# zju3dv/EnvGS

Hardware: AMD Instinct MI355X
Metric: train iters/s (fwd+bwd of the render hot path + Adam step, one 800x800 view per GPU per iter) + render Mpix/s (higher is better)
Workload: dtype f32

## Files before the change

### envgs_amd/csrc/trace_surfel_bwd.hip

```cpp
#include "trace_common.h"

namespace envgs {

#define ENVGS_LDS_FENCE() do { __builtin_amdgcn_s_waitcnt(0xc07f); __builtin_amdgcn_sched_barrier(0); } while (0)
#ifndef ENVGS_BS_GROUP
#define ENVGS_BS_GROUP 15
#endif
constexpr int BS_GROUP = ENVGS_BS_GROUP;
static_assert(BS_GROUP <= 16, "stage() assigns four lanes per entry");
#ifndef ENVGS_BSB_KO
#define ENVGS_BSB_KO 0
#endif

typedef float f32x4 __attribute__((ext_vector_type(4)));
constexpr int BT_PITCH = 96;
constexpr int RECW = 64;
template <bool RGBO, bool OTH>
__global__ void __attribute__((amdgpu_waves_per_eu(ENVGS_BSB_WAVES, ENVGS_BSB_WAVES))) __launch_bounds__(64)
batch_surfel_bwd(const TraceArgs A)
{
    static_assert(!(RGBO && OTH), "the colour-only form never touches `others`");
    __shared__ float4 sdat[2][BS_GROUP][16];
    __shared__ unsigned long long sdesc[2][BS_GROUP];
    __shared__ unsigned short kmat[2][BS_GROUP][64];
    __shared__ unsigned spb[2][BS_GROUP];
    __shared__ unsigned scn[2][BS_GROUP];
    __shared__ float btile[16][BT_PITCH];
    __shared__ float2 sox[2][BS_GROUP];
    const int lane = threadIdx.x;
    const int nb = (A.D + 1) * (A.D + 1);
    const int nbatch = (A.R + 63) >> 6;
    for (int slot = blockIdx.x; slot < nbatch; slot += gridDim.x) {
        const int batch = A.bwd_order ? (int)A.bwd_order[slot] : slot;
        if ((unsigned)batch >= (unsigned)nbatch) continue;
        const int base = batch << 6;
        const int copy = batch & (NCOPY - 1);
        const int r = ray_of(A, base + lane);
        const bool valid = r < A.R && A.hit_cnt[r < A.R ? r : 0] <= A.cap;
        const int rr = r < A.R ? r : 0;
        float basis[16], Box, Boy, Boz, Bdx, Bdy, Bdz, gR0, gR1, gR2, gD, gA, gN0, gN1, gN2, gX0, gX1, Fsum;
        {
            BwdRay B;
            bwd_load_ray(A, rr, B);
#pragma unroll
            for (int k = 0; k < 16; k++) basis[k] = 0.f;
            sh_basis(A.D, B.ux, B.uy, B.uz, basis);
            if (A.M == 0) basis[0] = kC0;
            if (!(B.il > 0.0f && B.il < 3.0e38f)) {
#pragma unroll
                for (int k = 0; k < 16; k++) basis[k] = 0.f;
            }
            Box = B.ox; Boy = B.oy; Boz = B.oz; Bdx = B.dx; Bdy = B.dy; Bdz = B.dz;
            gR0 = B.gR0; gR1 = B.gR1; gR2 = B.gR2;
            if constexpr (RGBO) { gD = gA = gN0 = gN1 = gN2 = gX0 = gX1 = 0.f; }
            else { gD = B.gD; gA = B.gA; gN0 = B.gN0; gN1 = B.gN1; gN2 = B.gN2; gX0 = B.gX0; gX1 = B.gX1; }
            Fsum = bwd_final_dot(B);
        }
        float Areg[16];
        __syncthreads();
#pragma unroll
        for (int k = 0; k < 16; k++) btile[k][lane + 2 * k] = (valid && k < nb) ? basis[k] : (k == 0 ? kC0 : 0.f);
        __syncthreads();
#pragma unroll
        for (int sI = 0; sI < 16; sI++) Areg[sI] = btile[lane & 15][4 * sI + (lane >> 4) + 2 * (lane & 15)];
        float Acol[16];
#pragma unroll
        for (int q = 0; q < 16; q++) {
            const int k = 4 * (q & 3) + (lane >> 4);
            Acol[q] = btile[k][16 * (q >> 2) + (lane & 15) + 2 * k];
        }
        __syncthreads();
        f32x4 SkM[4];
#pragma unroll
        for (int k = 0; k < 4; k++) SkM[k] = f32x4{0.f, 0.f, 0.f, 0.f};
        float dO0 = 0.f, dO1 = 0.f, dO2 = 0.f, dD0 = 0.f, dD1 = 0.f, dD2 = 0.f;
        const float4 *state = A.state + state_row0(A, min(base + lane, A.R - 1), rr);
        const char *plane1 = reinterpret_cast<const char *>(A.state + A.state_plane);
        size_t rstart, region;
        batch_region(A, batch, rstart, region);
        const unsigned long long *ent = A.entries + rstart;
        const unsigned *prs = A.pairs + rstart;
        const int D = A.n_entries[2 * batch], NE = D + A.n_entries[2 * batch + 1];
        unsigned poff = 0u;
        auto stage = [&](int g, int buf) {
            const int el = lane >> 2, part = lane & 3;
            const int e = g * BS_GROUP + el;
            const bool elv = el < BS_GROUP;
            unsigned long long d = 0ull;
            if (elv && e < NE) {
                d = e < D ? ent[e] : ent[region - 1 - (size_t)(e - D)];
                const int sid = (int)(d & 0xFFFFFFull);
                sdat[buf][el][part] = A.srec[(size_t)sid * 4 + part];
                if (A.M == 16 && A.f16) {
                    const uint2 *s2 = reinterpret_cast<const uint2 *>(reinterpret_cast<const __half *>(A.shs) + (size_t)sid * 48);
#pragma unroll
                    for (int q = 0; q < 3; q++) {
                        const uint2 h = s2[part * 3 + q];
                        float4 x = make_float4(__half2float(__ushort_as_half((unsigned short)(h.x & 0xFFFFu))), __half2float(__ushort_as_half((unsigned short)(h.x >> 16))),
                                               __half2float(__ushort_as_half((unsigned short)(h.y & 0xFFFFu))), __half2float(__ushort_as_half((unsigned short)(h.y >> 16))));
                        const int i0 = (part * 3 + q) * 4;
                        if (i0 + 0 >= nb * 3) x.x = 0.f;
                        if (i0 + 1 >= nb * 3) x.y = 0.f;
                        if (i0 + 2 >= nb * 3) x.z = 0.f;
                        if (i0 + 3 >= nb * 3) x.w = 0.f;
                        sdat[buf][el][4 + part * 3 + q] = x;
                    }
                } else if (A.M == 16) {
                    const float4 *s4 = reinterpret_cast<const float4 *>(A.shs + (size_t)sid * 48);
#pragma unroll
                    for (int q = 0; q < 3; q++) {
                        float4 x = s4[part * 3 + q];
                        const int i0 = (part * 3 + q) * 4;
                        if (i0 + 0 >= nb * 3) x.x = 0.f;
                        if (i0 + 1 >= nb * 3) x.y = 0.f;
                        if (i0 + 2 >= nb * 3) x.z = 0.f;
                        if (i0 + 3 >= nb * 3) x.w = 0.f;
                        sdat[buf][el][4 + part * 3 + q] = x;
                    }
                } else {
                    const Feat fsh = Feat{A.shs, A.f16 != 0}.at(A.M > 0 ? (size_t)sid * A.M * 3 : 0), fcol = Feat{A.colors, A.f16 != 0}.at(A.M > 0 ? 0 : (size_t)sid * 3);
#pragma unroll
                    for (int q = 0; q < 3; q++) {
                        float v[4];
#pragma unroll
                        for (int c = 0; c < 4; c++) {
                            const int idx = (part * 3 + q) * 4 + c;
                            v[c] = A.M > 0 ? (idx < nb * 3 ? fsh[idx] : 0.f) : (idx < 3 ? fcol[idx] : 0.f);
                        }
                        sdat[buf][el][4 + part * 3 + q] = make_float4(v[0], v[1], v[2], v[3]);
                    }
                }
                if (part == 0) {
                    const size_t ci = (size_t)sid * NCOPY + copy;
                    const unsigned rec = A.surf_off[ci] - A.surf_cnt[ci] + (unsigned)(d >> 32);
                    sdesc[buf][el] = (d & 0x3FFFFFFFull) | ((unsigned long long)rec << 32);
                    if constexpr (OTH) sox[buf][el] = reinterpret_cast<const float2 *>(A.others)[sid];
                }
            }
            if (part == 0 && elv) scn[buf][el] = e < NE ? (unsigned)((d >> 24) & 63ull) + 1u : 0u;
            if (lane * 32 < BS_GROUP * 128) {
                uint4 *km = reinterpret_cast<uint4 *>(&kmat[buf][0][0]);
                km[lane * 2] = make_uint4(0u, 0u, 0u, 0u); km[lane * 2 + 1] = make_uint4(0u, 0u, 0u, 0u);
            }
            __syncthreads();
            unsigned pref[BS_GROUP + 1];
            pref[0] = 0u;
#pragma unroll
            for (int q = 0; q < BS_GROUP; q++) pref[q + 1] = pref[q] + scn[buf][q];
            unsigned tab_before = 0u;
#pragma unroll
            for (int q = 0; q < BS_GROUP; q++) {
                const int eq = g * BS_GROUP + q;
                if (lane == q) spb[buf][q] = eq < D ? poff + tab_before : (unsigned)(region - 1 - (size_t)(eq - D));
                if (eq < D) tab_before += scn[buf][q];
            }
            __syncthreads();
            const unsigned total = pref[BS_GROUP];
            for (unsigned q = lane; q < total; q += 64) {
                int eli = 0;
#pragma unroll
                for (int t = 1; t < BS_GROUP; t++) eli += q >= pref[t] ? 1 : 0;
                const unsigned pr = prs[spb[buf][eli] + (q - pref[eli])];
                kmat[buf][eli][pr >> 16] = (unsigned short)((pr & 0xFFFFu) + 1u);
            }
            poff += tab_before;
        };
        __syncthreads();
        stage(0, 0);
        for (int g = 0; g * BS_GROUP < NE; g++) {
            const int buf = g & 1;
            __syncthreads();
            if ((g + 1) * BS_GROUP < NE) stage(g + 1, buf ^ 1);
            const int ne = min(BS_GROUP, NE - g * BS_GROUP);
            int k1 = valid ? (int)kmat[buf][0][lane] : 0;
            float4 st0, st1 = make_float4(0.f, 0.f, 0.f, 0.f), st2 = make_float4(0.f, 0.f, 0.f, 0.f);
            auto fetch_state = [&](const int k) {
                const float4 *sp = k > 0 ? state + (size_t)(k - 1) : A.state;
                if (ENVGS_BSB_KO & 8) st0 = make_float4(0.5f, 0.1f, 0.1f, 0.1f); else st0 = sp[0];
                if constexpr (!RGBO) {
                    if (ENVGS_BSB_KO & 4) return;
                    if constexpr (OTH) {
                        typedef float f3 __attribute__((ext_vector_type(3), aligned(4)));
                        const float *q = reinterpret_cast<const float *>(plane1 + (size_t)(sp - A.state) * 24);
                        const f3 a = *reinterpret_cast<const f3 *>(q); st1.x = a.x; st1.y = a.y; st1.z = a.z;
                        if (!(ENVGS_BSB_KO & 2)) { const f3 b = *reinterpret_cast<const f3 *>(q + 3); st1.w = b.x; st2.x = b.y; st2.y = b.z; }
                    } else st1 = *reinterpret_cast<const float4 *>(plane1 + (size_t)(sp - A.state) * 16);
                }
            };
            fetch_state(k1);
            auto entry = [&]<int e5>(const int el) __attribute__((always_inline)) {
                const unsigned long long d = sdesc[buf][el];
                const int sid = (int)(d & 0xFFFFFFull);
                const unsigned long long rec = d >> 32;
                const bool act = k1 > 0;
                float gw[16];
#pragma unroll
                for (int n = 0; n < 16; n++) gw[n] = 0.f;
                [[maybe_unused]] float gx1 = 0.f;
#define BT(n) btile[3 * e5 + (n)][lane + 2 * (3 * e5 + (n))]
                if (A.M > 0 && e5 == 0) {
                    const int nrun = min(5, ne - el);
                    const int kk = lane >> 4, nn = lane & 15, ee = nn / 3, c2 = nn - 3 * ee;
                    f32x4 cc0 = {0.f, 0.f, 0.f, 0.f}, cc1 = cc0, cc2 = cc0, cc3 = cc0;
                    float bvc[4];
#pragma unroll
                    for (int ks = 0; ks < 4; ks++) {
                        bvc[ks] = 0.f;
                        if (nn < 15 && ee < nrun) bvc[ks] = reinterpret_cast<const float *>(&sdat[buf][el + ee][4])[(4 * ks + kk) * 3 + c2];
                    }
                    ENVGS_LDS_FENCE();
#pragma unroll
                    for (int ks = 0; ks < 4; ks++) {
                        cc0 = __builtin_amdgcn_mfma_f32_16x16x4f32(Acol[ks], bvc[ks], cc0, 0, 0, 0);
                        cc1 = __builtin_amdgcn_mfma_f32_16x16x4f32(Acol[4 + ks], bvc[ks], cc1, 0, 0, 0);
                        cc2 = __builtin_amdgcn_mfma_f32_16x16x4f32(Acol[8 + ks], bvc[ks], cc2, 0, 0, 0);
                        cc3 = __builtin_amdgcn_mfma_f32_16x16x4f32(Acol[12 + ks], bvc[ks], cc3, 0, 0, 0);
                    }
                    if (nn < 15) {
                        float *trow = &btile[nn][0];
#pragma unroll
                        for (int i = 0; i < 4; i++) {
                            const int j = 4 * kk + i + 2 * nn;
                            trow[j] = cc0[i]; trow[j + 16] = cc1[i]; trow[j + 32] = cc2[i]; trow[j + 48] = cc3[i];
                        }
                    }
                }
                if (act) {
                    const float4 s0 = sdat[buf][el][0], s1 = sdat[buf][el][1], s2 = sdat[buf][el][2], s3 = sdat[buf][el][3];
                    const SurfHit h = hit_surfel(s0, s1, s2, s3, Box, Boy, Boz, Bdx, Bdy, Bdz);
                    float col[3]; bool cl[3] = {false, false, false};
                    if (A.M > 0) {
                        const float rc[3] = {BT(0), BT(1), BT(2)};
#pragma unroll
                        for (int c = 0; c < 3; c++) { const float v = rc[c] + 0.5f; cl[c] = v < 0.f; col[c] = cl[c] ? 0.f : v; }
                    } else { const float4 x = sdat[buf][el][4]; col[0] = x.x; col[1] = x.y; col[2] = x.z; }
                    float x0 = 0.f, x1 = 0.f;
                    if constexpr (OTH) { const float2 xo = sox[buf][el]; x0 = xo.x; x1 = xo.y; }
                    const float alpha = h.alpha, w = alpha * st0.x;
                    const float sgn = h.denom < 0.0f ? 1.0f : -1.0f;
                    const float nf0 = sgn * s3.x, nf1 = sgn * s3.y, nf2 = sgn * s3.z;
                    const float inv1m = __builtin_amdgcn_rcpf(1.0f - alpha);
                    const float dLa = alpha_grad_from_state(RGBO, gR0, gR1, gR2, gD, gA, gN0, gN1, gN2, gX0, gX1, Fsum, col, h.t, nf0, nf1, nf2, x0, x1,
                                                            alpha, inv1m, st0, st1, st2.x, st2.y);
                    if constexpr (OTH) { gw[15] = w * gX0; gx1 = w * gX1; }
                    BT(0) = cl[0] ? 0.f : w * gR0; BT(1) = cl[1] ? 0.f : w * gR1; BT(2) = cl[2] ? 0.f : w * gR2;
                    float e0, e1, e2;
                    hit_geometry_grad(s0, s1, s2, s3, h, Box, Boy, Boz, Bdx, Bdy, Bdz, w, sgn, dLa, gD, gN0, gN1, gN2, A.mod,
                                      __builtin_amdgcn_rcpf(s1.w), __builtin_amdgcn_rcpf(s2.w), __builtin_amdgcn_rcpf(h.denom), gw, e0, e1, e2);
                    dO0 += e0; dO1 += e1; dO2 += e2;
                    dD0 += h.t * e0; dD1 += h.t * e1; dD2 += h.t * e2;
                } else {
                    BT(0) = 0.f; BT(1) = 0.f; BT(2) = 0.f;
                }
#undef BT
                if (el + 1 < ne) {
                    k1 = valid ? (int)kmat[buf][el + 1][lane] : 0;
                    fetch_state(k1);
                }
                {
                    if constexpr (OTH && !(ENVGS_BSB_KO & 1)) {
                        float g20[20];
#pragma unroll
                        for (int n = 0; n < 20; n++) g20[n] = n < 15 ? gw[n] : 0.f;
                        g20[15] = gw[15]; g20[16] = gx1;
                        const float gsum = wave_transpose_reduce<5>(g20, lane);
                        const int word = (lane & 15) + 5 * (lane >> 4);
                        if ((lane & 15) < 5 && word < 15 && rec < A.num_records) A.records[rec * RECW + 48 + word] = gsum;
                        if ((lane & 15) < 5 && (word == 15 || word == 16) && A.dothers) atomic_add_f32(A.dothers + 2 * sid + (word - 15), gsum);
                    } else {
                        const float gsum = wave_transpose_reduce<4>(gw, lane);
                        const int word = (lane & 15) + 4 * (lane >> 4);
                        if ((lane & 15) < 4 && word < 15 && rec < A.num_records) A.records[rec * RECW + 48 + word] = gsum;
                    }
                }
                if (e5 == 4 || el + 1 == ne) {
                    f32x4 acc4 = {0.f, 0.f, 0.f, 0.f}, accB = acc4, accC = acc4, accD = acc4;
                    {
                        const int n = lane & 15, j = lane >> 4;
                        const float *brow = &btile[n][0];
                        const int rot = 2 * n + j;
                        float bvr[16];
#pragma unroll
                        for (int sI = 0; sI < 16; sI++) bvr[sI] = brow[4 * sI + rot];
                        ENVGS_LDS_FENCE();
#pragma unroll
                        for (int sI = 0; sI < 16; sI += 4) {
                            acc4 = __builtin_amdgcn_mfma_f32_16x16x4f32(Areg[sI], bvr[sI], acc4, 0, 0, 0);
                            accB = __builtin_amdgcn_mfma_f32_16x16x4f32(Areg[sI + 1], bvr[sI + 1], accB, 0, 0, 0);
                            accC = __builtin_amdgcn_mfma_f32_16x16x4f32(Areg[sI + 2], bvr[sI + 2], accC, 0, 0, 0);
                            accD = __builtin_amdgcn_mfma_f32_16x16x4f32(Areg[sI + 3], bvr[sI + 3], accD, 0, 0, 0);
                        }
                    }
                    acc4 = (acc4 + accB) + (accC + accD);
                    const int n = lane & 15, mrow = (lane >> 4) * 4, er = n / 3, cc = n - 3 * er;
                    if (n < 15 && er <= e5) {
                        const unsigned long long rc = sdesc[buf][el - e5 + er] >> 32;
                        if (rc < A.num_records) {
                            float *ro = A.records + rc * RECW;
                            if (A.M > 0) { ro[(mrow + 0) * 3 + cc] = acc4[0]; ro[(mrow + 1) * 3 + cc] = acc4[1]; ro[(mrow + 2) * 3 + cc] = acc4[2]; ro[(mrow + 3) * 3 + cc] = acc4[3]; }
                            else if (mrow == 0) ro[cc] = acc4[0] * (1.0f / kC0);
                        }
                    }
                    if (A.M > 0) {
                        const int kk = lane >> 4, nn = lane & 15;
                        float bvs[4], avs[16];
#pragma unroll
                        for (int ks = 0; ks < 4; ks++) {
                            const int col = 4 * ks + kk, ee = col / 3, c2 = col - 3 * ee;
                            bvs[ks] = 0.f;
                            if (col < 15 && ee <= e5) bvs[ks] = reinterpret_cast<const float *>(&sdat[buf][el - e5 + ee][4])[nn * 3 + c2];
                            const float *arow = &btile[col][0];
#pragma unroll
                            for (int rb = 0; rb < 4; rb++) avs[4 * ks + rb] = arow[16 * rb + nn + 2 * col];
                        }
                        ENVGS_LDS_FENCE();
#pragma unroll
                        for (int ks = 0; ks < 4; ks++)
#pragma unroll
                            for (int rb = 0; rb < 4; rb++)
                                SkM[rb] = __builtin_amdgcn_mfma_f32_16x16x4f32(avs[4 * ks + rb], bvs[ks], SkM[rb], 0, 0, 0);
                    }
                }
            };
            for (int el = 0; el < ne; el += 5) {
                entry.template operator()<0>(el);
                if (el + 1 >= ne) break;
                entry.template operator()<1>(el + 1);
                if (el + 2 >= ne) break;
                entry.template operator()<2>(el + 2);
                if (el + 3 >= ne) break;
                entry.template operator()<3>(el + 3);
                if (el + 4 >= ne) break;
                entry.template operator()<4>(el + 4);
            }
        }
        __syncthreads();
#pragma unroll
        for (int rb = 0; rb < 4; rb++)
#pragma unroll
            for (int i = 0; i < 4; i++) btile[lane & 15][16 * rb + 4 * (lane >> 4) + i] = SkM[rb][i];
        __syncthreads();
        if (valid) {
            BwdRay B;
            bwd_load_ray(A, r, B);
            BwdAcc acc;
            bwd_init_acc(acc);
            acc.dO0 = dO0; acc.dO1 = dO1; acc.dO2 = dO2; acc.dD0 = dD0; acc.dD1 = dD1; acc.dD2 = dD2;
#pragma unroll
            for (int k = 0; k < 16; k++) acc.Sk[k] = btile[k][lane];
            bwd_store_ray(A, r, B, acc);
        }
    }
}

template __global__ void __attribute__((amdgpu_waves_per_eu(ENVGS_BSB_WAVES, ENVGS_BSB_WAVES))) __launch_bounds__(64) batch_surfel_bwd<false, false>(const TraceArgs A);
template __global__ void __attribute__((amdgpu_waves_per_eu(ENVGS_BSB_WAVES, ENVGS_BSB_WAVES))) __launch_bounds__(64) batch_surfel_bwd<false, true>(const TraceArgs A);
template __global__ void __attribute__((amdgpu_waves_per_eu(ENVGS_BSB_WAVES, ENVGS_BSB_WAVES))) __launch_bounds__(64) batch_surfel_bwd<true, false>(const TraceArgs A);

__global__ void __launch_bounds__(256)
sparse_hits_bwd(const TraceArgs A, const int rgbo)
{
    const unsigned filed = __hip_atomic_load(A.counter + ENVGS_CTR_SPARSE_FILED,__ATOMIC_RELAXED, __HIP_MEMORY_SCOPE_AGENT);
    const unsigned n = filed < A.sparse_cap ? filed : A.sparse_cap;
    const int nb = (A.D + 1) * (A.D + 1);
    for (unsigned i = blockIdx.x * 256u + threadIdx.x; i < n; i += gridDim.x * 256u) {
        const uint4 e = A.sparse[i];
        bool ok = e.x < (unsigned)A.R && e.z < (unsigned)A.P;
        int r = A.R;
        if (ok) {
            r = ray_of(A, (int)e.x);
            ok = r < A.R && A.hit_cnt[r] <= A.cap && e.y < (unsigned)A.n_used[r];
        }
        if (ok) {
            const size_t ci0 = (size_t)e.z * NCOPY + (((int)e.x >> 6) & (NCOPY - 1));
            ok = (unsigned long long)(A.surf_off[ci0] - A.surf_cnt[ci0]) + (unsigned long long)e.w < A.num_records;
        }
        if (!ok) { atomicAdd(A.counter + ENVGS_CTR_SPARSE_SKIPPED, 1u); continue; }
        const int slot = (int)e.x, k = (int)e.y, sid = (int)e.z;
        BwdRay B;
        bwd_load_ray(A, r, B);
        float basis[16];
#pragma unroll
        for (int q = 0; q < 16; q++) basis[q] = 0.f;
        sh_basis(A.D, B.ux, B.uy, B.uz, basis);
        const size_t row = state_row0(A, slot, r) + (size_t)k;
        const float4 st0 = A.state[row];
        float4 st1 = make_float4(0.f, 0.f, 0.f, 0.f);
        float sx0 = 0.f, sx1 = 0.f;
        if (!rgbo) {
            if (A.has_others) {
                const float *q = reinterpret_cast<const float *>(state_row1(A, row));
                st1 = make_float4(q[0], q[1], q[2], q[3]); sx0 = q[4]; sx1 = q[5];
            } else st1 = *reinterpret_cast<const float4 *>(state_row1(A, row));
        }
        const float4 *sr = A.srec + (size_t)sid * 4;
        const float4 s0 = sr[0], s1 = sr[1], s2 = sr[2], s3 = sr[3];
        const SurfHit h = hit_surfel(s0, s1, s2, s3, B.ox, B.oy, B.oz, B.dx, B.dy, B.dz);
        float shv[48];
        float col[3]; bool cl[3];
        if (A.M > 0) {
            load_sh(A, sid, nb, shv);
            sh_colour_clamped(basis, shv, 16, col, cl);
        } else surfel_color(A, sid, basis, col, cl);
        const float x0 = (!rgbo && A.has_others) ? A.others[2 * sid] : 0.f, x1 = (!rgbo && A.has_others) ? A.others[2 * sid + 1] : 0.f;
        const float alpha = h.alpha, w = alpha * st0.x;
        const float sgn = h.denom < 0.0f ? 1.0f : -1.0f;
        const float nf0 = sgn * s3.x, nf1 = sgn * s3.y, nf2 = sgn * s3.z;
        const float dLa = alpha_grad_from_state(rgbo != 0, B.gR0, B.gR1, B.gR2, B.gD, B.gA, B.gN0, B.gN1, B.gN2, B.gX0, B.gX1, bwd_final_dot(B), col, h.t,
                                                nf0, nf1, nf2, x0, x1, alpha, 1.0f / (1.0f - alpha), st0, st1, sx0, sx1);
        const float dc[3] = {cl[0] ? 0.f : w * B.gR0, cl[1] ? 0.f : w * B.gR1, cl[2] ? 0.f : w * B.gR2};
        float gw[16], e0, e1, e2;
        hit_geometry_grad(s0, s1, s2, s3, h, B.ox, B.oy, B.oz, B.dx, B.dy, B.dz, w, sgn, dLa, B.gD, B.gN0, B.gN1, B.gN2, A.mod,
                          1.0f / s1.w, 1.0f / s2.w, 1.0f / h.denom, gw, e0, e1, e2);
        gw[15] = 0.f;
        const int copy = (slot >> 6) & (NCOPY - 1);
        const size_t ci = (size_t)sid * NCOPY + copy;
        const unsigned long long rec = (unsigned long long)(A.surf_off[ci] - A.surf_cnt[ci]) + (unsigned long long)e.w;
        {
            float4 *ro = reinterpret_cast<float4 *>(A.records + rec * RECW);
            if (A.M > 0) {
#pragma unroll
                for (int q = 0; q < 12; q++) {
                    float v[4];
#pragma unroll
                    for (int j = 0; j < 4; j++) { const int wd = 4 * q + j; v[j] = basis[wd / 3] * dc[wd % 3]; }
                    ro[q] = make_float4(v[0], v[1], v[2], v[3]);
                }
            } else ro[0] = make_float4(dc[0], dc[1], dc[2], 0.f);
#pragma unroll
            for (int q = 0; q < 4; q++) ro[12 + q] = make_float4(gw[4 * q], gw[4 * q + 1], gw[4 * q + 2], gw[4 * q + 3]);
        }
        float dd0 = 0.f, dd1 = 0.f, dd2 = 0.f;
        if (A.M > 0) {
            float bgx[16], bgy[16], bgz[16];
            sh_basis_grad(A.D, B.ux, B.uy, B.uz, bgx, bgy, bgz);
#pragma unroll
            for (int q = 0; q < 16; q++) {
                const float sk = q < nb ? shv[q * 3] * dc[0] + shv[q * 3 + 1] * dc[1] + shv[q * 3 + 2] * dc[2] : 0.f;
                dd0 += bgx[q] * sk; dd1 += bgy[q] * sk; dd2 += bgz[q] * sk;
            }
        }
        float f[3];
        ray_dir_grad(B, dd0, dd1, dd2, f);
        atomic_add_f32(A.dray_o + 3 * r, e0); atomic_add_f32(A.dray_o + 3 * r + 1, e1); atomic_add_f32(A.dray_o + 3 * r + 2, e2);
        atomic_add_f32(A.dray_d + 3 * r, h.t * e0 + f[0]); atomic_add_f32(A.dray_d + 3 * r + 1, h.t * e1 + f[1]); atomic_add_f32(A.dray_d + 3 * r + 2, h.t * e2 + f[2]);
        if (!rgbo && A.has_others && A.dothers) { atomic_add_f32(A.dothers + 2 * sid, w * B.gX0); atomic_add_f32(A.dothers + 2 * sid + 1, w * B.gX1); }
    }
}

constexpr int RED_LONG = 96;
__device__ __forceinline__ void reduce_store(const TraceArgs &A, const int sid, const int q, const int nb, const float *v)
{
#pragma unroll
    for (int e = 0; e < 4; e++) {
        const int wd = 4 * q + e;
        if (wd < 48) {
            float *o = nullptr;
            if (A.M > 0) { if (wd / 3 < nb) o = A.dshs + (size_t)sid * A.M * 3 + wd; }
            else if (wd < 3) o = A.dcolors + (size_t)sid * 3 + wd;
            if (o) *o = A.reduce_adds ? *o + v[e] : v[e];
        } else if (wd < 63) {
            float *o = A.geo_rec + (size_t)sid * GEO + (wd - 48);
            *o = A.reduce_adds ? *o + v[e] : v[e];
        }
    }
}
__global__ void __launch_bounds__(256)
reduce_surfel_records(const TraceArgs A)
{
    __shared__ int longs[64];
    __shared__ int nlong;
    __shared__ float4 part[16][16];
    const int sub = threadIdx.x >> 4, q = threadIdx.x & 15;
    const int nb = (A.D + 1) * (A.D + 1);
    const float4 *rp = reinterpret_cast<const float4 *>(A.records) + q;
    if (threadIdx.x == 0) nlong = 0;
    __syncthreads();
    for (int sid0 = blockIdx.x * 16; sid0 < A.P; sid0 += gridDim.x * 16) {
        const int sid = sid0 + sub;
        if (sid >= A.P) continue;
        const unsigned end = A.surf_off[(size_t)sid * NCOPY + NCOPY - 1];
        const unsigned begin = A.surf_off[(size_t)sid * NCOPY] - A.surf_cnt[(size_t)sid * NCOPY];
        if (end <= begin) continue;
        if (end - begin > (unsigned)RED_LONG) {
            int k = 0;
            if (q == 0) k = atomicAdd(&nlong, 1);
            k = __shfl(k, 0, 16);
            if (k < 64) { if (q == 0) longs[k] = sid; continue; }
        }
        const unsigned long long hi = end < A.num_records ? end : A.num_records;
        float4 a0 = make_float4(0.f, 0.f, 0.f, 0.f), a1 = a0, a2 = a0, a3 = a0;
        unsigned long long i = begin;
        for (; i + 4 <= hi; i += 4) {
            const float4 x0 = rp[i * 16], x1 = rp[(i + 1) * 16], x2 = rp[(i + 2) * 16], x3 = rp[(i + 3) * 16];
            a0.x += x0.x; a0.y += x0.y; a0.z += x0.z; a0.w += x0.w; a1.x += x1.x; a1.y += x1.y; a1.z += x1.z; a1.w += x1.w;
            a2.x += x2.x; a2.y += x2.y; a2.z += x2.z; a2.w += x2.w; a3.x += x3.x; a3.y += x3.y; a3.z += x3.z; a3.w += x3.w;
        }
        for (; i < hi; i++) { const float4 x0 = rp[i * 16]; a0.x += x0.x; a0.y += x0.y; a0.z += x0.z; a0.w += x0.w; }
        const float v[4] = {(a0.x + a1.x) + (a2.x + a3.x), (a0.y + a1.y) + (a2.y + a3.y), (a0.z + a1.z) + (a2.z + a3.z), (a0.w + a1.w) + (a2.w + a3.w)};
        reduce_store(A, sid, q, nb, v);
    }
    __syncthreads();
    const int nl = nlong < 64 ? nlong : 64;
    for (int k = 0; k < nl; k++) {
        const int sid = longs[k];
        const unsigned end = A.surf_off[(size_t)sid * NCOPY + NCOPY - 1];
        const unsigned begin = A.surf_off[(size_t)sid * NCOPY] - A.surf_cnt[(size_t)sid * NCOPY];
        const unsigned long long hi = end < A.num_records ? end : A.num_records;
        float4 a0 = make_float4(0.f, 0.f, 0.f, 0.f), a1 = a0;
        unsigned long long i = (unsigned long long)begin + sub;
        for (; i + 16 < hi; i += 32) {
            const float4 x0 = rp[i * 16], x1 = rp[(i + 16) * 16];
            a0.x += x0.x; a0.y += x0.y; a0.z += x0.z; a0.w += x0.w; a1.x += x1.x; a1.y += x1.y; a1.z += x1.z; a1.w += x1.w;
        }
        if (i < hi) { const float4 x0 = rp[i * 16]; a0.x += x0.x; a0.y += x0.y; a0.z += x0.z; a0.w += x0.w; }
        __syncthreads();
        part[sub][q] = make_float4(a0.x + a1.x, a0.y + a1.y, a0.z + a1.z, a0.w + a1.w);
        __syncthreads();
        if (sub == 0) {
            float v[4] = {0.f, 0.f, 0.f, 0.f};
#pragma unroll
            for (int g = 0; g < 16; g++) { const float4 x = part[g][q]; v[0] += x.x; v[1] += x.y; v[2] += x.z; v[3] += x.w; }
            reduce_store(A, sid, q, nb, v);
        }
    }
}

__global__ void __launch_bounds__(256)
finish_surfel_grads(int P, const float *__restrict__ rots, const float *__restrict__ geo_rec, float *__restrict__ dmeans,
                    float *__restrict__ dscales, float *__restrict__ dopac, float *__restrict__ drots, float *__restrict__ dgrads3D)
{
    const int i = blockIdx.x * 256 + threadIdx.x;
    if (i >= P) return;
    const float q0 = rots[4 * i], q1 = rots[4 * i + 1], q2 = rots[4 * i + 2], q3 = rots[4 * i + 3];
    const float qq = q0 * q0 + q1 * q1 + q2 * q2 + q3 * q3;
    const float inv = qq > 0.0f ? 1.0f / sqrtf(qq) : 0.0f;
    const float r = q0 * inv, x = q1 * inv, y = q2 * inv, z = q3 * inv;
    const float *g = geo_rec + (size_t)i * GEO;
    const float *rr = g + 3;
#define VR(a, b) rr[(b) * 3 + (a)]
    drots[4 * i + 0] = 2.f * (x * (VR(2, 1) - VR(1, 2)) + y * (VR(0, 2) - VR(2, 0)) + z * (VR(1, 0) - VR(0, 1)));
    drots[4 * i + 1] = 2.f * (-2.f * x * (VR(1, 1) + VR(2, 2)) + y * (VR(1, 0) + VR(0, 1)) + z * (VR(2, 0) + VR(0, 2)) + r * (VR(2, 1) - VR(1, 2)));
    drots[4 * i + 2] = 2.f * (x * (VR(1, 0) + VR(0, 1)) - 2.f * y * (VR(0, 0) + VR(2, 2)) + z * (VR(2, 1) + VR(1, 2)) + r * (VR(0, 2) - VR(2, 0)));
    drots[4 * i + 3] = 2.f * (x * (VR(2, 0) + VR(0, 2)) + y * (VR(2, 1) + VR(1, 2)) - 2.f * z * (VR(0, 0) + VR(1, 1)) + r * (VR(1, 0) - VR(0, 1)));
#undef VR
    dmeans[3 * i] = g[0]; dmeans[3 * i + 1] = g[1]; dmeans[3 * i + 2] = g[2];
    dscales[2 * i] = g[12]; dscales[2 * i + 1] = g[13];
    dopac[i] = g[14];
    if (dgrads3D) { dgrads3D[3 * i] = g[0]; dgrads3D[3 * i + 1] = g[1]; dgrads3D[3 * i + 2] = g[2]; }
}


}
```

Before: 140.4.

## Replace block barriers with wave fences and rebuild staging via readlane prefix

Since the kernel runs one 64-lane wavefront per block, every __syncthreads is swapped for a wavefront-scope fence plus an LDS waitcnt. The stage() routine is rebuilt around this. The next group's entry descriptor is prefetched one group ahead. Per-entry hit counts are broadcast with readlane instead of going through shared scn/spb arrays and two barriers, and each lane loads its own pair index per entry directly, so the serial prefix-sum scatter loop goes away. Global loads for srec, surf_off/cnt and others are hoisted ahead of the LDS writes. Optional cycle-counter instrumentation is added behind a macro, and so are scratch scripts that check results match the previous build bit for bit. The risk is correctness if any block ever has more than one wave, and extra register pressure from the pr[] array.

```diff
diff --git a/envgs_amd/csrc/trace_surfel_bwd.hip b/envgs_amd/csrc/trace_surfel_bwd.hip
--- a/envgs_amd/csrc/trace_surfel_bwd.hip
+++ b/envgs_amd/csrc/trace_surfel_bwd.hip
@@ -10,6 +10,17 @@
 static_assert(BS_GROUP <= 16, "stage() assigns four lanes per entry");
 #ifndef ENVGS_BSB_KO
 #define ENVGS_BSB_KO 0
+#endif
+
+#define ENVGS_WAVE_SYNC() do { __builtin_amdgcn_fence(__ATOMIC_ACQ_REL, "wavefront"); ENVGS_LDS_FENCE(); } while (0)
+#ifndef ENVGS_BSB_TIMING
+#define ENVGS_BSB_TIMING 0
+#endif
+#if ENVGS_BSB_TIMING
+#define ENVGS_BSB_LAP(bucket) do { __builtin_amdgcn_sched_barrier(0); const unsigned long long t_ = __builtin_readcyclecounter(); \
+                                   bucket += t_ - cyc_last; cyc_last = t_; __builtin_amdgcn_sched_barrier(0); } while (0)
+#else
+#define ENVGS_BSB_LAP(bucket) do { } while (0)
 #endif
 
 typedef float f32x4 __attribute__((ext_vector_type(4)));
@@ -23,13 +34,14 @@
     __shared__ float4 sdat[2][BS_GROUP][16];
     __shared__ unsigned long long sdesc[2][BS_GROUP];
     __shared__ unsigned short kmat[2][BS_GROUP][64];
-    __shared__ unsigned spb[2][BS_GROUP];
-    __shared__ unsigned scn[2][BS_GROUP];
     __shared__ float btile[16][BT_PITCH];
     __shared__ float2 sox[2][BS_GROUP];
     const int lane = threadIdx.x;
     const int nb = (A.D + 1) * (A.D + 1);
     const int nbatch = (A.R + 63) >> 6;
+#if ENVGS_BSB_TIMING
+    unsigned long long cyc_pro = 0, cyc_stage = 0, cyc_entry = 0, cyc_sync = 0, cyc_last = __builtin_readcyclecounter();
+#endif
     for (int slot = blockIdx.x; slot < nbatch; slot += gridDim.x) {
         const int batch = A.bwd_order ? (int)A.bwd_order[slot] : slot;
         if ((unsigned)batch >= (unsigned)nbatch) continue;
@@ -57,10 +69,10 @@
             Fsum = bwd_final_dot(B);
         }
         float Areg[16];
-        __syncthreads();
+        ENVGS_WAVE_SYNC();
 #pragma unroll
         for (int k = 0; k < 16; k++) btile[k][lane + 2 * k] = (valid && k < nb) ? basis[k] : (k == 0 ? kC0 : 0.f);
-        __syncthreads();
+        ENVGS_WAVE_SYNC();
 #pragma unroll
         for (int sI = 0; sI < 16; sI++) Areg[sI] = btile[lane & 15][4 * sI + (lane >> 4) + 2 * (lane & 15)];
         float Acol[16];
@@ -69,7 +81,7 @@
             const int k = 4 * (q & 3) + (lane >> 4);
             Acol[q] = btile[k][16 * (q >> 2) + (lane & 15) + 2 * k];
         }
-        __syncthreads();
+        ENVGS_WAVE_SYNC();
         f32x4 SkM[4];
 #pragma unroll
         for (int k = 0; k < 4; k++) SkM[k] = f32x4{0.f, 0.f, 0.f, 0.f};
@@ -82,15 +94,44 @@
         const unsigned *prs = A.pairs + rstart;
         const int D = A.n_entries[2 * batch], NE = D + A.n_entries[2 * batch + 1];
         unsigned poff = 0u;
+        auto fetch_desc = [&](const int g) -> unsigned long long {
+            const int e = g * BS_GROUP + (lane >> 2);
+            const bool ok = (lane >> 2) < BS_GROUP && e < NE;
+            const unsigned long long *p = ok ? ent + (e < D ? (size_t)e : region - 1 - (size_t)(e - D)) : A.entries;
+            const unsigned long long d = *p;
+            return ok ? d : 0ull;
+        };
+        unsigned long long dnext = fetch_desc(0);
         auto stage = [&](int g, int buf) {
             const int el = lane >> 2, part = lane & 3;
             const int e = g * BS_GROUP + el;
             const bool elv = el < BS_GROUP;
-            unsigned long long d = 0ull;
+            const unsigned long long d = dnext;
+            dnext = fetch_desc(g + 1);
+            if (lane * 32 < BS_GROUP * 128) {
+                uint4 *km = reinterpret_cast<uint4 *>(&kmat[buf][0][0]);
+                km[lane * 2] = make_uint4(0u, 0u, 0u, 0u); km[lane * 2 + 1] = make_uint4(0u, 0u, 0u, 0u);
+            }
+            const unsigned hits = (elv && e < NE) ? (unsigned)((d >> 24) & 63ull) + 1u : 0u;
+            unsigned pr[BS_GROUP];
+            unsigned tab_before = 0u;
+#pragma unroll
+            for (int q = 0; q < BS_GROUP; q++) {
+                const unsigned cq = (unsigned)__builtin_amdgcn_readlane((int)hits, 4 * q);
+                const int eq = g * BS_GROUP + q;
+                const unsigned first = eq < D ? poff + tab_before : (unsigned)(region - 1 - (size_t)(eq - D));
+                if (eq < D) tab_before += cq;
+                pr[q] = *((unsigned)lane < cq ? prs + first + lane : A.pairs);
+            }
+            poff += tab_before;
+            __builtin_amdgcn_fence(__ATOMIC_ACQ_REL, "wavefront"); __builtin_amdgcn_sched_barrier(0);
             if (elv && e < NE) {
-                d = e < D ? ent[e] : ent[region - 1 - (size_t)(e - D)];
                 const int sid = (int)(d & 0xFFFFFFull);
-                sdat[buf][el][part] = A.srec[(size_t)sid * 4 + part];
+                const size_t ci = (size_t)sid * NCOPY + copy;
+                const float4 r4 = A.srec[(size_t)sid * 4 + part];
+                const unsigned s_off = A.surf_off[ci], s_cnt = A.surf_cnt[ci];
+                float2 s_ox = make_float2(0.f, 0.f);
+                if constexpr (OTH) s_ox = reinterpret_cast<const float2 *>(A.others)[sid];
                 if (A.M == 16 && A.f16) {
                     const uint2 *s2 = reinterpret_cast<const uint2 *>(reinterpret_cast<const __half *>(A.shs) + (size_t)sid * 48);
 #pragma unroll
@@ -130,47 +171,28 @@
                         sdat[buf][el][4 + part * 3 + q] = make_float4(v[0], v[1], v[2], v[3]);
                     }
                 }
+                sdat[buf][el][part] = r4;
                 if (part == 0) {
-                    const size_t ci = (size_t)sid * NCOPY + copy;
-                    const unsigned rec = A.surf_off[ci] - A.surf_cnt[ci] + (unsigned)(d >> 32);
+                    const unsigned rec = s_off - s_cnt + (unsigned)(d >> 32);
                     sdesc[buf][el] = (d & 0x3FFFFFFFull) | ((unsigned long long)rec << 32);
-                    if constexpr (OTH) sox[buf][el] = reinterpret_cast<const float2 *>(A.others)[sid];
+                    if constexpr (OTH) sox[buf][el] = s_ox;
                 }
             }
-            if (part == 0 && elv) scn[buf][el] = e < NE ? (unsigned)((d >> 24) & 63ull) + 1u : 0u;
-            if (lane * 32 < BS_GROUP * 128) {
-                uint4 *km = reinterpret_cast<uint4 *>(&kmat[buf][0][0]);
-                km[lane * 2] = make_uint4(0u, 0u, 0u, 0u); km[lane * 2 + 1] = make_uint4(0u, 0u, 0u, 0u);
-            }
-            __syncthreads();
-            unsigned pref[BS_GROUP + 1];
-            pref[0] = 0u;
-#pragma unroll
-            for (int q = 0; q < BS_GROUP; q++) pref[q + 1] = pref[q] + scn[buf][q];
-            unsigned tab_before = 0u;
-#pragma unroll
-            for (int q = 0; q < BS_GROUP; q++) {
-                const int eq = g * BS_GROUP + q;
-                if (lane == q) spb[buf][q] = eq < D ? poff + tab_before : (unsigned)(region - 1 - (size_t)(eq - D));
-                if (eq < D) tab_before += scn[buf][q];
-            }
-            __syncthreads();
-            const unsigned total = pref[BS_GROUP];
-            for (unsigned q = lane; q < total; q += 64) {
-                int eli = 0;
-#pragma unroll
-                for (int t = 1; t < BS_GROUP; t++) eli += q >= pref[t] ? 1 : 0;
-                const unsigned pr = prs[spb[buf][eli] + (q - pref[eli])];
-                kmat[buf][eli][pr >> 16] = (unsigned short)((pr & 0xFFFFu) + 1u);
-            }
-            poff += tab_before;
+#pragma unroll
+            for (int q = 0; q < BS_GROUP; q++)
+                if ((unsigned)lane < (unsigned)__builtin_amdgcn_readlane((int)hits, 4 * q)) kmat[buf][q][pr[q] >> 16] = (unsigned short)((pr[q] & 0xFFFFu) + 1u);
         };
-        __syncthreads();
+        ENVGS_WAVE_SYNC();
+        ENVGS_BSB_LAP(cyc_pro);
         stage(0, 0);
+        ENVGS_BSB_LAP(cyc_stage);
         for (int g = 0; g * BS_GROUP < NE; g++) {
             const int buf = g & 1;
-            __syncthreads();
+            ENVGS_BSB_LAP(cyc_entry);
+            ENVGS_WAVE_SYNC();
+            ENVGS_BSB_LAP(cyc_sync);
             if ((g + 1) * BS_GROUP < NE) stage(g + 1, buf ^ 1);
+            ENVGS_BSB_LAP(cyc_stage);
             const int ne = min(BS_GROUP, NE - g * BS_GROUP);
             int k1 = valid ? (int)kmat[buf][0][lane] : 0;
             float4 st0, st1 = make_float4(0.f, 0.f, 0.f, 0.f), st2 = make_float4(0.f, 0.f, 0.f, 0.f);
@@ -334,12 +356,13 @@
                 entry.template operator()<4>(el + 4);
             }
         }
-        __syncthreads();
+        ENVGS_BSB_LAP(cyc_entry);
+        ENVGS_WAVE_SYNC();
 #pragma unroll
         for (int rb = 0; rb < 4; rb++)
 #pragma unroll
             for (int i = 0; i < 4; i++) btile[lane & 15][16 * rb + 4 * (lane >> 4) + i] = SkM[rb][i];
-        __syncthreads();
+        ENVGS_WAVE_SYNC();
         if (valid) {
             BwdRay B;
             bwd_load_ray(A, r, B);
@@ -350,7 +373,15 @@
             for (int k = 0; k < 16; k++) acc.Sk[k] = btile[k][lane];
             bwd_store_ray(A, r, B, acc);
         }
+        ENVGS_BSB_LAP(cyc_pro);
     }
+#if ENVGS_BSB_TIMING
+    if (lane == 0) {
+        unsigned long long *tot = reinterpret_cast<unsigned long long *>(A.counter + ENVGS_CTR_TOTALS);
+        atomicAdd(tot + ENVGS_TOT_ROUNDS, cyc_pro); atomicAdd(tot + ENVGS_TOT_COOP_EXPAND, cyc_stage);
+        atomicAdd(tot + ENVGS_TOT_COOP_WALK, cyc_entry); atomicAdd(tot + ENVGS_TOT_COOP_WAIT, cyc_sync);
+    }
+#endif
 }
 
 template __global__ void __attribute__((amdgpu_waves_per_eu(ENVGS_BSB_WAVES, ENVGS_BSB_WAVES))) __launch_bounds__(64) batch_surfel_bwd<false, false>(const TraceArgs A);
diff --git a/scratch/bsb_same_forward.py b/scratch/bsb_same_forward.py
--- /dev/null
+++ b/scratch/bsb_same_forward.py
@@ -0,0 +1,72 @@
+import ctypes, sys, os
+sys.path.insert(0, os.path.dirname(os.path.dirname(os.path.abspath(__file__))))
+import torch
+from envgs_amd import _lib
+_lib.LIB_PATH = os.path.abspath(sys.argv[1])
+from envgs_amd import synth, tracing, fused, envgs_step
+import diff_surfel_tracing as tpkg
+import diff_surfel_rasterization_wet_ch05 as pkg
+
+tag = "same_forward"
+dev = torch.device("cuda:0")
+lib = _lib.load()
+H = W = 800
+g = synth.base_gaussians(300000, seed=0, device=dev)
+ge = synth.env_gaussians(163840, seed=1, device=dev)
+cam = synth.orbit_camera(0, n_views=8, H=H, W=W, fx=1111.1, device=dev)
+rays = synth.get_rays(cam)
+envgs_step.FUSED["on"] = True
+base = {k: g[k] for k in ("means3D", "shs", "opacities", "scales", "rotations")}
+base["specular"] = g["specular"]; base["roughness"] = g["roughness"]
+tracer = tpkg.SurfelTracer()
+with torch.no_grad():
+    out = envgs_step.envgs_forward(pkg, tpkg, tracer, cam, rays, base, {k: ge[k] for k in base if k in ge}, torch.zeros(3, device=dev), torch.zeros(3, device=dev), torch.tensor([3], device=dev))
+ro, rd = out["ref_o"].reshape(-1, 3).contiguous(), out["ref_d"].reshape(-1, 3).contiguous()
+
+NAMES = []
+while lib.envgs_prof_kernel_name(len(NAMES)):
+    NAMES.append(lib.envgs_prof_kernel_name(len(NAMES)).decode())
+
+
+def drain():
+    r = {}
+    for k, nm in enumerate(NAMES):
+        t_, c_ = ctypes.c_double(0), ctypes.c_int(0)
+        lib.envgs_prof_read(k, ctypes.byref(t_), ctypes.byref(c_))
+        if c_.value:
+            r[nm] = (t_.value / c_.value, c_.value)
+    return r
+
+
+def totals(counters):
+    w = counters.cpu()
+    v = w[_lib.CTR_TOTALS:_lib.CTR_TOTALS + 2 * _lib.TOT_COUNT].view(torch.int64)
+    return [int(v[k]) for k in (_lib.TOT_ROUNDS, _lib.TOT_COOP_EXPAND, _lib.TOT_COOP_WALK, _lib.TOT_COOP_WAIT)]
+
+
+ts = tpkg.SurfelTracingSettings(image_height=H, image_width=W, tanfovx=cam.tanfovx, tanfovy=cam.tanfovy, bg=torch.zeros(3, device=dev), scale_modifier=1.0,
+                                viewmatrix=cam.world_view_transform, projmatrix=cam.full_proj_transform, sh_degree=3, campos=cam.camera_center,
+                                prefiltered=False, debug=False, max_trace_depth=0, specular_threshold=0.0)
+v, f = fused.surfel_quads(ge["means3D"], ge["scales"], ge["rotations"])
+nodes, _ = tracing.build_bvh(v, ge["opacities"])
+caps = tracing.CapState()
+caps.colour_only = True
+for it in range(4):
+    outs, saved = tracing.trace_forward(nodes, ro, rd, ge["means3D"], ge["shs"], None, None, ge["opacities"], ge["scales"], ge["rotations"], ts, False, caps=caps)
+    torch.cuda.synchronize()
+tc = tracing.last_trace_counts(); ent = sum(tracing.last_entry_counts())
+R = ro.shape[0]
+g_rgb = (torch.randn(R, 3, generator=torch.Generator().manual_seed(5)) / R).to(dev)
+gr = (g_rgb, None, None, None, None)
+print("sparse hits filed:", tc["sparse_hits"], "max_list", tc["max_list"], "cap", tc["cap"], "rays without rows", tc["rays_without_rows"], flush=True)
+def run():
+    out = tracing.trace_backward(saved, *gr)
+    tracing.join_deferred_gradients(); torch.cuda.synchronize()
+    return {k: v.clone() for k, v in out.items() if v is not None}
+new1 = run(); new2 = run()
+_lib._libs["product"] = _lib._open(os.path.abspath(sys.argv[2]))
+old1 = run(); old2 = run()
+for k in new1:
+    m = float(old1[k].abs().max())
+    print("%-14s change vs change %-9s parent vs parent %-9s change vs parent %-9s max|a-b|/max|b| %.3e" % (k, "bit-equal" if torch.equal(new1[k], new2[k]) else "differs",
+          "bit-equal" if torch.equal(old1[k], old2[k]) else "differs", "bit-equal" if torch.equal(new1[k], old1[k]) else "differs", float((new1[k] - old1[k]).abs().max()) / max(m, 1e-30)), flush=True)
diff --git a/scratch/bsb_stage_split.py b/scratch/bsb_stage_split.py
--- /dev/null
+++ b/scratch/bsb_stage_split.py
@@ -0,0 +1,78 @@
+import ctypes, sys, os
+sys.path.insert(0, os.path.dirname(os.path.dirname(os.path.abspath(__file__))))
+import torch
+from envgs_amd import _lib
+_lib.LIB_PATH = os.path.abspath(sys.argv[1])
+from envgs_amd import synth, tracing, fused, envgs_step
+import diff_surfel_tracing as tpkg
+import diff_surfel_rasterization_wet_ch05 as pkg
+
+tag = sys.argv[2] if len(sys.argv) > 2 else os.path.basename(sys.argv[1])
+dev = torch.device("cuda:0")
+lib = _lib.load()
+H = W = 800
+g = synth.base_gaussians(300000, seed=0, device=dev)
+ge = synth.env_gaussians(163840, seed=1, device=dev)
+cam = synth.orbit_camera(0, n_views=8, H=H, W=W, fx=1111.1, device=dev)
+rays = synth.get_rays(cam)
+envgs_step.FUSED["on"] = True
+base = {k: g[k] for k in ("means3D", "shs", "opacities", "scales", "rotations")}
+base["specular"] = g["specular"]; base["roughness"] = g["roughness"]
+tracer = tpkg.SurfelTracer()
+with torch.no_grad():
+    out = envgs_step.envgs_forward(pkg, tpkg, tracer, cam, rays, base, {k: ge[k] for k in base if k in ge}, torch.zeros(3, device=dev), torch.zeros(3, device=dev), torch.tensor([3], device=dev))
+ro, rd = out["ref_o"].reshape(-1, 3).contiguous(), out["ref_d"].reshape(-1, 3).contiguous()
+
+NAMES = []
+while lib.envgs_prof_kernel_name(len(NAMES)):
+    NAMES.append(lib.envgs_prof_kernel_name(len(NAMES)).decode())
+
+
+def drain():
+    r = {}
+    for k, nm in enumerate(NAMES):
+        t_, c_ = ctypes.c_double(0), ctypes.c_int(0)
+        lib.envgs_prof_read(k, ctypes.byref(t_), ctypes.byref(c_))
+        if c_.value:
+            r[nm] = (t_.value / c_.value, c_.value)
+    return r
+
+
+def totals(counters):
+    w = counters.cpu()
+    v = w[_lib.CTR_TOTALS:_lib.CTR_TOTALS + 2 * _lib.TOT_COUNT].view(torch.int64)
+    return [int(v[k]) for k in (_lib.TOT_ROUNDS, _lib.TOT_COOP_EXPAND, _lib.TOT_COOP_WALK, _lib.TOT_COOP_WAIT)]
+
+
+ts = tpkg.SurfelTracingSettings(image_height=H, image_width=W, tanfovx=cam.tanfovx, tanfovy=cam.tanfovy, bg=torch.zeros(3, device=dev), scale_modifier=1.0,
+                                viewmatrix=cam.world_view_transform, projmatrix=cam.full_proj_transform, sh_degree=3, campos=cam.camera_center,
+                                prefiltered=False, debug=False, max_trace_depth=0, specular_threshold=0.0)
+v, f = fused.surfel_quads(ge["means3D"], ge["scales"], ge["rotations"])
+nodes, _ = tracing.build_bvh(v, ge["opacities"])
+caps = tracing.CapState()
+caps.colour_only = True
+for it in range(4):
+    outs, saved = tracing.trace_forward(nodes, ro, rd, ge["means3D"], ge["shs"], None, None, ge["opacities"], ge["scales"], ge["rotations"], ts, False, caps=caps)
+    torch.cuda.synchronize()
+tc = tracing.last_trace_counts(); ent = sum(tracing.last_entry_counts())
+R = ro.shape[0]
+g_rgb = (torch.randn(R, 3, generator=torch.Generator().manual_seed(5)) / R).to(dev)
+gr = (g_rgb, None, None, None, None)
+for _ in range(3):
+    tracing.trace_backward(saved, *gr)
+torch.cuda.synchronize()
+lib.envgs_prof_enable(1); drain()
+for _ in range(10):
+    tracing.trace_backward(saved, *gr)
+torch.cuda.synchronize()
+lib.envgs_prof_enable(0)
+ms = drain().get("trace.batch_surfel_bwd", (float("nan"), 0))[0]
+print("%s rays %d hits %.2f M entries %.3f M (%.1f hits/entry)  batch_surfel_bwd<true,false> %.4f ms per launch" % (tag, R, tc["hits"] / 1e6, ent / 1e6, tc["hits"] / max(ent, 1), ms), flush=True)
+t0 = totals(saved.counters)
+tracing.trace_backward(saved, *gr)
+torch.cuda.synchronize()
+d = [b - a for a, b in zip(t0, totals(saved.counters))]
+if sum(d):
+    s = float(sum(d))
+    print("%s wavefront cycles of one launch: prologue/epilogue %d (%.1f %%)  stage() %d (%.1f %%)  entry bodies %d (%.1f %%)  group-top sync %d (%.1f %%)  | per entry: stage %.0f  body %.0f" % (
+        tag, d[0], 100 * d[0] / s, d[1], 100 * d[1] / s, d[2], 100 * d[2] / s, d[3], 100 * d[3] / s, d[1] / max(ent, 1), d[2] / max(ent, 1)), flush=True)
```

Result: faster. 145.7, median of 6 (+3.8%).
